# paradigmxyz/reth

Hardware: NVIDIA H100
Metric: keccak256_digests_per_sec (higher is better)
Workload: dtype u64

## Files before the change

reth_b200/csrc/tk_branch.cuh:

```cuda

struct ChildInfo {
    uint32_t id;
    uint32_t nib;
    uint32_t meta;
};

template <bool COHERENT = false>
__device__ __forceinline__ ChildInfo fetch_child(const ForestDev &f, uint32_t j0, uint32_t c) {
    ChildInfo ci;
    if (c == 0) {
        uint32_t g = f.gap_sorted[j0];
        ci.id = f.E[g - 1];
        ci.nib = f.nibs[g] >> 4;
    } else {
        uint32_t g = f.gap_sorted[j0 + c - 1];
        ci.id = f.S[g];
        ci.nib = f.nibs[g] & 15;
    }
    if (COHERENT) ci.meta = ci.id < f.n ? __ldcg(f.leaf_meta + ci.id) : __ldcg(f.node_meta + (ci.id - (uint32_t)f.n));
    else ci.meta = ci.id < f.n ? f.leaf_meta[ci.id] : f.node_meta[ci.id - (uint32_t)f.n];
    return ci;
}

template <class W>
// ... 118 lines not shown
        const uint32_t t3 = (sw & 1) ? (i >= 1 ? T2[i - 1] : 0u) : T2[i];
        if (base_word + i < 34) m[base_word + i] ^= t3;
    }
}

__device__ __forceinline__ void branch23_words(const uint32_t (&r0)[8], const uint32_t (&r1)[8], const uint32_t (&r2)[8], uint32_t n0,
                                               uint32_t n1, uint32_t n2, bool three, uint32_t (&m)[34]) {
#pragma unroll
    for (int w = 0; w < 34; w++) {
        uint32_t two_v = w == 0 ? 0x808051f8u : (w < 20 ? 0x80808080u : (w == 20 ? 0x01808080u : 0u));
        uint32_t three_v = w == 0 ? 0x808071f8u : (w < 28 ? 0x80808080u : (w == 28 ? 0x01808080u : 0u));
        if (w == 33) {
            two_v = 0x80000000u;
            three_v = 0x80000000u;
        }
        m[w] = two_v == three_v ? two_v : (three ? three_v : two_v);
    }
    xor_child33(m, 0, r0, n0, true);
    xor_child33(m, 8, r1, n1, true);
    xor_child33(m, 16, r2, n2, three);
}

template <int BLOCK>
__device__ __forceinline__ uint32_t thread_finish_node(Strip<BLOCK> &s, uint32_t (&ref)[8], uint32_t meta, int pd, int d,
                                                       const uint8_t *key, uint32_t &hashed, uint32_t &exts) {
    if (pd + 1 >= d) return meta;
    s.reset();
    uint32_t elen = encode_extension(s, key, (uint32_t)(pd + 1), (uint32_t)d, ref, meta);
    exts++;
    return strip_to_ref(s, elen, pd < 0, ref, hashed) | META_EXT;
}

template <int BLOCK, int MAXC, bool COHERENT>
__device__ __forceinline__ void thread_build_node(Strip<BLOCK> &s, uint32_t *smem, const ForestDev &f, uint32_t v, int d,
                                                  uint32_t &hashed, uint32_t &exts, uint32_t (&ref)[8]) {
    s.init(smem);
    uint32_t j0 = f.node_start[v], k = f.node_start[v + 1] - j0;
    if (k + 1 > (uint32_t)MAXC) k = MAXC - 1;
    uint32_t state_mask, tree_mask, hash_mask, l, r;
    uint32_t meta;
    bool done = false;
    if constexpr (MAXC == 3 && !COHERENT) {
        const uint32_t n = (uint32_t)f.n;
        const uint32_t g0 = f.gap_sorted[j0], g1 = k >= 2 ? f.gap_sorted[j0 + 1] : g0;
        uint32_t id[3], nb[3], mt[3];
        id[0] = f.E[g0 - 1];
        nb[0] = f.nibs[g0] >> 4;
        id[1] = f.S[g0];
        nb[1] = f.nibs[g0] & 15;
        id[2] = k >= 2 ? f.S[g1] : id[1];
        nb[2] = k >= 2 ? (uint32_t)(f.nibs[g1] & 15) : 15u;
#pragma unroll
        for (int c = 0; c < 3; c++) mt[c] = id[c] < n ? f.leaf_meta[id[c]] : f.node_meta[id[c] - n];
        const bool three = k >= 2;
        if (k >= 1 && ((mt[0] | mt[1] | (three ? mt[2] : 0u)) & META_LEN) == 0) {
            uint32_t rr[3][8];
#pragma unroll
            for (int c = 0; c < 3; c++)
                load32_nc(id[c] < n ? f.leaf_ref + 32 * (uint64_t)id[c] : f.node_ref + 32 * (uint64_t)(id[c] - n), rr[c]);
            state_mask = tree_mask = hash_mask = 0;
#pragma unroll
            for (int c = 0; c < 3; c++) {
                if (c < 2 || three) {
                    const uint32_t bit = 1u << nb[c];
                    state_mask |= bit;
                    if (id[c] >= n || (mt[c] & META_ISNODE)) {
                        if (!(mt[c] & META_EXT)) hash_mask |= bit;
                        if (mt[c] & META_STORED) tree_mask |= bit;
                    }
                }
// ... 4 lines not shown
            uint32_t m[34];
            branch23_words(rr[0], rr[1], rr[2], nb[0], nb[1], nb[2], three, m);
            uint64_t a[25];
#pragma unroll
            for (int q = 0; q < 17; q++) a[q] = ((uint64_t)m[2 * q + 1] << 32) | m[2 * q];
#pragma unroll
            for (int q = 17; q < 25; q++) a[q] = 0;
            keccak_f1600_final(a);
#pragma unroll
            for (int q = 0; q < 4; q++) {
                ref[2 * q] = (uint32_t)a[q];
                ref[2 * q + 1] = (uint32_t)(a[q] >> 32);
            }
            hashed++;
            meta = 0;
            done = true;
        }
    }
    uint32_t len = 0;
    if (!done) len = encode_branch_u<BLOCK, MAXC, COHERENT>(s, f, j0, k, state_mask, tree_mask, hash_mask, l, r);
    const int pd = parent_depth(f, l, r);
    if (!done) meta = strip_to_ref(s, len, pd < 0 && pd + 1 >= d, ref, hashed);
    meta = thread_finish_node(s, ref, meta, pd, d, f.keys + 32 * (uint64_t)l, hashed, exts);
    bool stored = (tree_mask | hash_mask) != 0;
    if (stored) meta |= META_STORED;
    store32(f.node_ref + 32 * (uint64_t)v, ref);
    f.node_meta[v] = (uint8_t)meta;
    f.node_l[v] = l;
    f.node_r[v] = r;
    f.node_masks[v] = make_ushort4((unsigned short)state_mask, (unsigned short)tree_mask, (unsigned short)hash_mask,
                                   (unsigned short)d);
    f.S[l] = (uint32_t)f.n + v;
    f.E[r] = (uint32_t)f.n + v;
}

struct PrefetchedNode3 {
    uint32_t v, j0, k;
    uint32_t g0, g1;
    uint32_t id[3], nb[3], mt[3];
    uint32_t rr[3][8];
    uint32_t nl, nr;
    bool valid;
};

template <int BLOCK>
__device__ __forceinline__ void pf3_stage_a(const ForestDev &f, const uint32_t *__restrict__ node_order, uint64_t p, uint32_t pos_hi,
                                            PrefetchedNode3 &x) {
    x.valid = p < pos_hi;
    if (x.valid) {
        x.v = __ldg(node_order + p);
        x.j0 = f.node_start[x.v];
        x.k = f.node_start[x.v + 1] - x.j0;
    }
}
__device__ __forceinline__ void pf3_stage_b(const ForestDev &f, PrefetchedNode3 &x) {
    if (x.valid) {
        x.g0 = f.gap_sorted[x.j0];
        x.g1 = x.k >= 2 ? f.gap_sorted[x.j0 + 1] : x.g0;
    }
}
__device__ __forceinline__ void pf3_stage_c(const ForestDev &f, PrefetchedNode3 &x) {
    if (x.valid) {
        const uint32_t nib0 = f.nibs[x.g0], nib1 = f.nibs[x.g1];
        x.id[0] = f.E[x.g0 - 1];
        x.id[1] = f.S[x.g0];
        x.id[2] = x.k >= 2 ? f.S[x.g1] : x.id[1];
// ... 70 lines not shown
            keccak_rounds<17, 23>(a);
            keccak_round(a, 0x8000000080008008ULL);
#pragma unroll
            for (int q = 0; q < 4; q++) {
                ref[2 * q] = (uint32_t)a[q];
                ref[2 * q + 1] = (uint32_t)(a[q] >> 32);
            }
            hashed++;
            int pdl = depth_of(lpl), pdr = depth_of(lpr);
            int pd = pdl > pdr ? pdl : pdr;
            meta = thread_finish_node(s, ref, 0u, pd, d, f.keys + 32 * (uint64_t)l, hashed, exts);
            if ((tree_mask | hash_mask) != 0) meta |= META_STORED;
            store32(f.node_ref + 32 * (uint64_t)v, ref);
            f.node_meta[v] = (uint8_t)meta;
            f.node_l[v] = l;
            f.node_r[v] = r;
            f.node_masks[v] = make_ushort4((unsigned short)state_mask, (unsigned short)tree_mask, (unsigned short)hash_mask,
                                           (unsigned short)d);
            f.S[l] = n + v;
            f.E[r] = n + v;
        } else {
            pf3_stage_b(f, nx);
            pf3_stage_c(f, nx);
            pf3_stage_d(f, nx);
            thread_build_node<BLOCK, 3, false>(s, smem, f, v, d, hashed, exts, ref);
        }
        cur = nx;
        p += step;
    }
    flush_counters(f.counters, hashed, exts);
}

template <int BLOCK, int MAXC>
__global__ void __launch_bounds__(BLOCK) branch_kernel(ForestDev f, const uint32_t *__restrict__ node_order,
                                                       uint32_t pos_lo, uint32_t pos_hi, int d) {
    extern __shared__ uint32_t smem[];
    if (*(volatile int *)f.err != B200_DEVERR_NONE) return;
    Strip<BLOCK> s;
    uint32_t hashed = 0, exts = 0;
    const uint32_t step = gridDim.x * BLOCK;
    for (uint64_t p64 = (uint64_t)pos_lo + blockIdx.x * BLOCK + threadIdx.x; p64 < pos_hi; p64 += step) {
        uint32_t ref[8];
        thread_build_node<BLOCK, MAXC, false>(s, smem, f, __ldg(node_order + p64), d, hashed, exts, ref);
    }
    flush_counters(f.counters, hashed, exts);
}
```

reth_b200/csrc/tk_dtrie.cuh:

```cuda

static __device__ __forceinline__ uint32_t dt_nib(const uint8_t *key, uint32_t i) { return key_nibble_mem(key, i); }

static __device__ __forceinline__ uint32_t dt_lcp(const uint8_t *a, const uint8_t *b, uint32_t from, uint32_t limit) {
    uint32_t i = from & ~1u;
    for (; i < limit; i += 2) {
        uint32_t x = a[i >> 1] ^ b[i >> 1];
        if (x) {
            uint32_t l = (x & 0xF0) ? i : i + 1;
            return l < limit ? l : limit;
        }
    }
    return limit;
}

static __device__ __forceinline__ void dt_copy32(uint8_t *dst, const uint8_t *src) {
    const uint4 *s = reinterpret_cast<const uint4 *>(src);
    uint4 *d = reinterpret_cast<uint4 *>(dst);
    d[0] = s[0];
    d[1] = s[1];
}
static __device__ __forceinline__ void dt_copy72(uint8_t *dst, const uint8_t *src) {
    const uint64_t *s = reinterpret_cast<const uint64_t *>(src);
    uint64_t *d = reinterpret_cast<uint64_t *>(dst);
#pragma unroll
// ... 761 lines not shown
                                                     uint32_t &hashed, uint32_t &exts, uint32_t (&ref)[8]) {
    s.init(smem);
    const int d = t.ndepth[v];
    uint32_t state_mask, tree_mask, hash_mask;
    const uint32_t payload = dt_branch_payload<true>(t, v, state_mask, tree_mask, hash_mask);
    dt_put_branch<true>(s, t, v, payload);
    const uint32_t par = t.nparent[v];
    const int pd = par == DT_NONE ? -1 : (int)t.ndepth[par];
    uint32_t meta = strip_to_ref(s, list_header_len(payload) + payload, pd < 0 && pd + 1 >= d, ref, hashed);
    meta = thread_finish_node(s, ref, meta, pd, d, t.nkey + 32 * (uint64_t)v, hashed, exts);
    if ((tree_mask | hash_mask) != 0) meta |= META_STORED;
    if ((t.nmeta[v] & META_STORED) && !(meta & META_STORED)) dt_record_removed(t, v);
    store32(t.nref + 32 * (uint64_t)v, ref);
    t.nmeta[v] = (uint8_t)meta;
    t.nmasks[v] = make_ushort4((unsigned short)state_mask, (unsigned short)tree_mask, (unsigned short)hash_mask, (unsigned short)d);
    t.built[atomicAdd(&t.g[DG_BUILT], 1u)] = v;
}

template <int BLOCK>
__global__ void __launch_bounds__(BLOCK) dt_wavefront_thread_kernel(DTrieDev t, const uint32_t *__restrict__ count_p,
                                                                   uint32_t *__restrict__ handoff_list,
                                                                   uint32_t *__restrict__ handoff_count, int split_depth) {
    extern __shared__ uint32_t smem[];
    if (*(volatile int *)t.err != B200_DEVERR_NONE) return;
    Strip<BLOCK> s;
    uint32_t hashed = 0, exts = 0;
    const uint32_t e = blockIdx.x * BLOCK + threadIdx.x;
    const uint32_t sd = e < *count_p ? t.seeds[e] : DT_NONE;
    if (sd != DT_NONE) {
        uint32_t ref[8];
        uint32_t p;
        if (sd & DT_LEAF) {
            const uint32_t x = sd & ~DT_LEAF;
            s.init(smem);
            p = t.lparent[x];
            const int pd = p == DT_NONE ? -1 : (int)t.ndepth[p];
            uint32_t k[8];
            load32_nc(t.lkey + 32 * (uint64_t)x, k);
            uint32_t len = t.account ? encode_leaf<Strip<BLOCK>, true>(s, k, pd, t.lval + 72 * (uint64_t)x,
                                                                        t.lsroot ? t.lsroot + 32 * (uint64_t)x : nullptr, t.err)
                                     : encode_leaf<Strip<BLOCK>, false>(s, k, pd, t.lval + 32 * (uint64_t)x, nullptr, t.err);
            uint32_t meta = strip_to_ref(s, len, pd < 0, ref, hashed);
            store32(t.lref + 32 * (uint64_t)x, ref);
            t.lmeta[x] = (uint8_t)meta;
        } else {
            dt_thread_build_node<BLOCK>(s, smem, t, sd, hashed, exts, ref);
            p = t.nparent[sd];
        }
        bool top = true;
        for (int hops = 0; p != DT_NONE; hops++) {
            if (hops > DT_MAX_HOPS) {
                atomicExch(t.err, B200_DEVERR_CORRUPT);
                top = false;
                break;
            }
            if ((int)t.ndepth[p] < split_depth) {
                __threadfence();
                handoff_list[atomicAdd(handoff_count, 1u)] = p;
                top = false;
                break;
            }
            __threadfence();
            bool last = atomicSub(&t.npending[p], 1u) == 1u;
            __threadfence();
            if (!last) {
                top = false;
                break;
            }
            dt_thread_build_node<BLOCK>(s, smem, t, p, hashed, exts, ref);
            p = t.nparent[p];
        }
        if (top) store32(t.top_out + (uint64_t)t.top_stride * dt_trie_of(t, sd), ref);
    }
    flush_counters(t.counters, hashed, exts);
}
// ... 56 lines not shown
```

reth_b200/csrc/tk_items.cuh:

```cuda
template <int BLOCK>
__global__ void __launch_bounds__(BLOCK) item_leaf_kernel(ForestDev f, ItemLeavesDev it, const uint8_t *__restrict__ values,
                                                          const uint8_t *__restrict__ storage_roots) {
    extern __shared__ uint32_t smem[];
    if (*(volatile int *)f.err == B200_DEVERR_UNSORTED || *(volatile int *)f.err == B200_DEVERR_BAD_OFFSETS) return;
    Strip<BLOCK> s;
    uint32_t hashed = 0, exts = 0;
    const uint32_t stride = it.account ? (uint32_t)sizeof(b200_account_dev) : 32u;
    const uint64_t step = (uint64_t)gridDim.x * BLOCK;
    for (uint64_t i = (uint64_t)blockIdx.x * BLOCK + threadIdx.x; i < f.n; i += step) {
        s.init(smem);
        const int pd = parent_depth(f, i, i);
        const uint32_t L = it.key_nibs[i];
        uint32_t ref[8], meta;
        if (L >= 64) {
            uint32_t k[8];
            load32(f.keys + 32 * i, k);
            const uint8_t *vp = values + (uint64_t)stride * i;
            uint32_t len = it.account ? encode_leaf<Strip<BLOCK>, true>(s, k, pd, vp, storage_roots ? storage_roots + 32 * i : nullptr, f.err)
                                      : encode_leaf<Strip<BLOCK>, false>(s, k, pd, vp, nullptr, f.err);
            meta = strip_to_ref(s, len, pd < 0, ref, hashed);
        } else {
            if (pd >= (int)L) atomicExch(f.err, B200_DEVERR_UNSORTED);
            {
                const uint2 *q = reinterpret_cast<const uint2 *>(values + (uint64_t)stride * i);
#pragma unroll
                for (int w = 0; w < 4; w++) {
                    uint2 t = __ldg(q + w);
                    ref[2 * w] = t.x;
                    ref[2 * w + 1] = t.y;
                }
            }
            meta = META_ISNODE | ((it.flags[i] & 1) ? META_STORED : 0u) |
                   thread_finish_node(s, ref, 0u, pd, (int)L, f.keys + 32 * i, hashed, exts);
        }
        store32(f.leaf_ref + 32 * i, ref);
        f.leaf_meta[i] = (uint8_t)meta;
        f.S[i] = (uint32_t)i;
        f.E[i] = (uint32_t)i;
    }
    flush_counters(f.counters, hashed, exts);
}

cudaError_t launch_item_leaves(const ForestDev &f, const ItemLeavesDev &it, const uint8_t *values, const uint8_t *storage_roots,
                               cudaStream_t st) {
    if (f.n == 0) return cudaSuccess;
    auto k = item_leaf_kernel<LEAF_BLOCK>;
    size_t smem = (size_t)LEAF_WORDS_ACCOUNT * LEAF_BLOCK * 4;
    k<<<persistent_grid(k, LEAF_BLOCK, smem, f.n), LEAF_BLOCK, smem, st>>>(f, it, values, storage_roots);
    return cudaGetLastError();
}
```

reth_b200/csrc/tk_launchers.cuh:

```cuda

static inline unsigned blocks_for(uint64_t n, unsigned block) { return (unsigned)((n + block - 1) / block); }

static int g_sms = 0;
static int sms() {
    if (!g_sms) {
        int dev = 0;
        cudaGetDevice(&dev);
        cudaDeviceGetAttribute(&g_sms, cudaDevAttrMultiProcessorCount, dev);
        if (g_sms <= 0) g_sms = 132;
    }
    return g_sms;
}

template <typename K>
static unsigned persistent_grid(K kernel, int block, size_t smem, uint64_t work_items) {
    static std::mutex mu;
    static std::unordered_map<const void *, int> cache;
    int per_sm;
    {
        std::lock_guard<std::mutex> g(mu);
        auto it = cache.find((const void *)kernel);
        if (it == cache.end()) {
            cudaFuncSetAttribute(kernel, cudaFuncAttributeMaxDynamicSharedMemorySize, (int)smem);
            per_sm = 1;
// ... 28 lines not shown
    return cudaGetLastError();
}
cudaError_t launch_gap_keys(const uint8_t *Lp, uint64_t G, uint16_t *key, uint32_t *val, uint32_t *unresolved, cudaStream_t st) {
    if (G == 0) return cudaSuccess;
    gap_keys_kernel<<<blocks_for(G, 256), 256, 0, st>>>(Lp, G, key, val, unresolved);
    return cudaGetLastError();
}
cudaError_t launch_bucket_offsets(const uint16_t *key_sorted, uint64_t G, uint32_t *bucket_off, cudaStream_t st) {
    bucket_offsets_kernel<<<1, 96, 0, st>>>(key_sorted, G, bucket_off);
    return cudaGetLastError();
}
cudaError_t launch_head_fix(const uint8_t *keys, uint16_t *key_sorted, const uint32_t *gap_sorted, const uint64_t *seg_offsets,
                            uint64_t n_segs, const uint32_t *unresolved, uint64_t G, cudaStream_t st) {
    if (G == 0) return cudaSuccess;
    head_fix_kernel<<<blocks_for(G, 256), 256, 0, st>>>(keys, key_sorted, gap_sorted, seg_offsets, n_segs, unresolved, G);
    return cudaGetLastError();
}
cudaError_t launch_level_ranges(uint32_t *node_start, const uint32_t *n_nodes_p, const uint32_t *bucket_off,
                                uint32_t *level_lo, cudaStream_t st) {
    level_ranges_kernel<<<1, 96, 0, st>>>(node_start, n_nodes_p, bucket_off, level_lo, node_start);
    return cudaGetLastError();
}

constexpr int LEAF_BLOCK = 128;
constexpr int LEAF_WORDS_STORAGE = 34;
constexpr int LEAF_WORDS_ACCOUNT = 68;
constexpr int BRANCH_BLOCK = 128;
constexpr int BRANCH_WORDS = 136;

cudaError_t launch_leaves(const ForestDev &f, bool account, const uint8_t *values, const uint8_t *storage_roots,
                          cudaStream_t st) {
    if (f.n == 0) return cudaSuccess;
    if (account) {
        auto k = leaf_kernel<LEAF_BLOCK, true>;
        size_t smem = (size_t)LEAF_WORDS_ACCOUNT * LEAF_BLOCK * 4;
        k<<<persistent_grid(k, LEAF_BLOCK, smem, f.n), LEAF_BLOCK, smem, st>>>(f, values, storage_roots);
    } else {
        auto k = leaf_storage_kernel<LEAF_BLOCK>;
        size_t smem = (size_t)LEAF_WORDS_STORAGE * LEAF_BLOCK * 4;
        k<<<blocks_for(f.n, LEAF_BLOCK), LEAF_BLOCK, smem, st>>>(f, values);
    }
    return cudaGetLastError();
}

template <int MAXC, int WORDS>
static cudaError_t launch_branch_class(const ForestDev &f, const uint32_t *node_order, uint32_t pos_lo, uint32_t pos_hi,
                                       int d, cudaStream_t st) {
    auto k = branch_kernel<BRANCH_BLOCK, MAXC>;
    size_t smem = (size_t)WORDS * BRANCH_BLOCK * 4;
    k<<<persistent_grid(k, BRANCH_BLOCK, smem, pos_hi - pos_lo), BRANCH_BLOCK, smem, st>>>(f, node_order, pos_lo,
                                                                                          pos_hi, d);
    return cudaGetLastError();
}

cudaError_t launch_branch_level(const ForestDev &f, const uint32_t *node_order, uint32_t pos_lo, uint32_t pos_hi,
                                int d, int cls, cudaStream_t st) {
    if (pos_hi <= pos_lo) return cudaSuccess;
    if (cls < 0) {
        constexpr int WARPS = 4;
        uint32_t cnt = pos_hi - pos_lo;
        unsigned blocks = (cnt + WARPS - 1) / WARPS;
        unsigned cap = (unsigned)sms() * 16;
        branch_warp_kernel<WARPS><<<blocks < cap ? blocks : cap, WARPS * 32, 0, st>>>(f, node_order, pos_lo, pos_hi, d);
        return cudaGetLastError();
    }
    switch (cls) {
        case 0: {
            auto k = branch3_pipelined_kernel<BRANCH_BLOCK>;
            size_t smem = (size_t)34 * BRANCH_BLOCK * 4;
// ... 220 lines not shown
```

reth_b200/csrc/tk_leaf.cuh:

```cuda

template <class W, bool ACCOUNT>
__device__ __forceinline__ uint32_t encode_leaf(W &s, const uint32_t (&k)[8], int pd, const uint8_t *val_ptr,
                                                const uint8_t *sroot_ptr, int *err) {
    uint32_t p = (uint32_t)(pd + 1);
    uint32_t m = 64 - p;
    uint32_t hp_len = 1 + (m >> 1);
    uint32_t hp_str = hp_len == 1 ? 1 : 1 + hp_len;
    uint32_t first = (p & 1) ? (0x30u | (byte_at(k, p >> 1) & 15)) : 0x20u;
    uint32_t b0 = (p + 1) >> 1;

    if (!ACCOUNT) {
        uint32_t v[8];
        load32(val_ptr, v);
        uint32_t z = leading_zero_bytes(v);
        if (z == 32) {
            atomicExch(err, B200_DEVERR_ZERO_VALUE);
            z = 31;
        }
        uint32_t vb = 32 - z;
        uint32_t fb = byte_at(v, z);
        bool single = vb == 1 && fb < 0x80;
        uint32_t rlp_v = single ? 1 : 1 + vb;
        uint32_t val_str = single ? 1 : 1 + rlp_v;
        uint32_t payload = hp_str + val_str;
        put_list_header(s, payload);
        if (hp_len > 1) s.byte(0x80 + hp_len);
        s.byte(first);
        s.tail32(k, b0);
        if (single) {
            s.byte(fb);
        } else {
            s.byte(0x80 + rlp_v);
            s.byte(0x80 + vb);
            s.tail32(v, z);
        }
        return list_header_len(payload) + payload;
    } else {
        const uint64_t *ap = reinterpret_cast<const uint64_t *>(val_ptr);
        uint64_t nonce = __ldg(ap);
        uint32_t bal[8], code[8], sroot[8];
        {
            const uint2 *q = reinterpret_cast<const uint2 *>(val_ptr + 8);
#pragma unroll
            for (int i = 0; i < 4; i++) {
                uint2 t = __ldg(q + i);
                bal[2 * i] = t.x;
                bal[2 * i + 1] = t.y;
            }
#pragma unroll
            for (int i = 0; i < 4; i++) {
                uint2 t = __ldg(q + 4 + i);
                code[2 * i] = t.x;
                code[2 * i + 1] = t.y;
            }
        }
        if (sroot_ptr) {
            load32_nc(sroot_ptr, sroot);
        } else {
            sroot[0] = 0x171fe856u; sroot[1] = 0xa655cc1bu; sroot[2] = 0xe64583ffu; sroot[3] = 0x6ef8c092u;
            sroot[4] = 0x1be0485bu; sroot[5] = 0xc0ad6c99u; sroot[6] = 0xb52f6201u; sroot[7] = 0x21b463e3u;
        }
        uint32_t nn = nonce == 0 ? 0 : (8 - (__clzll((long long)nonce) >> 3));
        uint32_t nonce_rlp = (nn == 0 || (nn == 1 && nonce < 0x80)) ? 1 : 1 + nn;
        uint32_t bz = leading_zero_bytes(bal);
        uint32_t bb = 32 - bz;
        uint32_t bfb = bb ? byte_at(bal, bz) : 0;
        uint32_t bal_rlp = (bb == 0 || (bb == 1 && bfb < 0x80)) ? 1 : 1 + bb;
        uint32_t inner_payload = nonce_rlp + bal_rlp + 66;
        uint32_t inner_total = 2 + inner_payload;
        uint32_t payload = hp_str + 2 + inner_total;
        s.byte(0xf8);
        s.byte(payload);
        if (hp_len > 1) s.byte(0x80 + hp_len);
        s.byte(first);
        s.tail32(k, b0);
        s.byte(0xb8);
        s.byte(inner_total);
        s.byte(0xf8);
        s.byte(inner_payload);
        if (nn == 0) {
            s.byte(0x80);
        } else {
            if (nonce_rlp > 1) s.byte(0x80 + nn);
            for (int i = (int)nn - 1; i >= 0; i--) s.byte((uint32_t)(nonce >> (8 * i)) & 0xff);
        }
        if (bb == 0) {
            s.byte(0x80);
        } else if (bal_rlp == 1) {
            s.byte(bfb);
        } else {
            s.byte(0x80 + bb);
            s.tail32(bal, bz);
        }
        s.byte(0xa0);
        s.words8(sroot);
        s.byte(0xa0);
        s.words8(code);
        return 2 + payload;
    }
// ... 53 lines not shown
    X[0] = (two ? 0u : (X[0] & 0xFF000000u)) | A;

    const uint32_t ov = a + 32 - b0, bv8 = 8 * (ov & 3), rel = (ov >> 2) - 5;
    uint32_t T0[13], T1[13];
#pragma unroll
    for (int i = 0; i < 13; i++) T0[i] = i < 10 ? __funnelshift_l(Y[i], Y[i + 1], bv8) : 0u;
#pragma unroll
    for (int i = 0; i < 13; i++) T1[i] = (rel & 2) ? (i >= 2 ? T0[i - 2] : 0u) : T0[i];
#pragma unroll
    for (int i = 0; i < 5; i++) mw[i] = X[i];
#pragma unroll
    for (int i = 0; i < 13; i++) {
        const uint32_t t2 = (rel & 1) ? (i >= 1 ? T1[i - 1] : 0u) : T1[i];
        mw[5 + i] = (5 + i < 9 ? X[5 + i] : 0u) | t2;
    }
    return (two ? 2u : 1u) + payload;
}

__device__ __forceinline__ void keccak_single_block18(const uint32_t (&mw)[18], uint32_t (&dig)[8]) {
    uint64_t a[25];
#pragma unroll
    for (int l = 0; l < 9; l++) a[l] = ((uint64_t)mw[2 * l + 1] << 32) | mw[2 * l];
#pragma unroll
    for (int l = 9; l < 25; l++) a[l] = 0;
    a[16] = 0x8000000000000000ULL;
    keccak_f1600_sparse_final(a);
#pragma unroll
    for (int l = 0; l < 4; l++) {
        dig[2 * l] = (uint32_t)a[l];
        dig[2 * l + 1] = (uint32_t)(a[l] >> 32);
    }
}

template <int BLOCK>
__device__ __forceinline__ uint32_t strip_to_ref(Strip<BLOCK> &s, uint32_t len, bool force_hash, uint32_t (&ref)[8],
                                                 uint32_t &hashed) {
    if (len >= 32 || force_hash) {
        uint32_t blocks = s.finish();
        strip_keccak(s, blocks, ref);
        hashed++;
        return 0;
    }
    while (s.nb != 0) s.byte(0);
#pragma unroll
    for (int i = 0; i < 8; i++) ref[i] = (uint32_t)i < s.nw ? s.read_word(i) : 0;
    return len;
}

template <int BLOCK, bool ACCOUNT>
__global__ void __launch_bounds__(BLOCK) leaf_kernel(ForestDev f, const uint8_t *__restrict__ values,
                                                     const uint8_t *__restrict__ storage_roots) {
    extern __shared__ uint32_t smem[];
    if (*(volatile int *)f.err == B200_DEVERR_UNSORTED || *(volatile int *)f.err == B200_DEVERR_BAD_OFFSETS) return;
    Strip<BLOCK> s;
    uint32_t hashed = 0;
    const uint64_t step = (uint64_t)gridDim.x * BLOCK;
    for (uint64_t i = (uint64_t)blockIdx.x * BLOCK + threadIdx.x; i < f.n; i += step) {
        s.init(smem);
        uint32_t k[8];
        load32(f.keys + 32 * i, k);
        const int pd = parent_depth(f, i, i);
        const uint8_t *vp = ACCOUNT ? values + (uint64_t)sizeof(b200_account_dev) * i : values + 32 * i;
        const uint8_t *sp = (ACCOUNT && storage_roots) ? storage_roots + 32 * i : nullptr;
        uint32_t len = encode_leaf<Strip<BLOCK>, ACCOUNT>(s, k, pd, vp, sp, f.err);
        uint32_t ref[8];
        uint32_t meta = strip_to_ref(s, len, pd < 0, ref, hashed);
        store32(f.leaf_ref + 32 * i, ref);
        f.leaf_meta[i] = (uint8_t)meta;
        f.S[i] = (uint32_t)i;
        f.E[i] = (uint32_t)i;
    }
    for (int o = 16; o; o >>= 1) hashed += __shfl_xor_sync(0xffffffffu, hashed, o);
    if ((threadIdx.x & 31) == 0 && hashed) atomicAdd(&f.counters[CNT_HASHED], (unsigned long long)hashed);
}

template <int BLOCK>
__global__ void __launch_bounds__(BLOCK) leaf_storage_kernel(ForestDev f, const uint8_t *__restrict__ values) {
    extern __shared__ uint32_t smem[];
    __shared__ uint32_t s_hashed;
    if (*(volatile int *)f.err == B200_DEVERR_UNSORTED || *(volatile int *)f.err == B200_DEVERR_BAD_OFFSETS) return;
    if (threadIdx.x == 0) s_hashed = 0;
    __syncthreads();
    const uint64_t i = (uint64_t)blockIdx.x * BLOCK + threadIdx.x;
    uint32_t hashed = 0;
    if (i < f.n) {
        uint32_t k[8], v[8], ref[8];
        load32(f.keys + 32 * i, k);
        load32(values + 32 * i, v);
        const int pd = parent_depth(f, i, i);
        uint32_t meta;
        if (pd >= 0 && pd <= 26) {
            uint32_t zi = 8, zword = 0;
#pragma unroll
            for (int w = 7; w >= 0; w--)
                if (v[w] != 0) {
                    zi = (uint32_t)w;
                    zword = v[w];
                }
            uint32_t z = 4 * zi + ((uint32_t)(__ffs((int)zword) - 1) >> 3);
            if (zi == 8) {
                atomicExch(f.err, B200_DEVERR_ZERO_VALUE);
                z = 31;
            }
            uint32_t mw[18];
            const uint32_t len = storage_leaf_words(k, v, (uint32_t)(pd + 1), z, mw);
            if (len >= 32) {
                keccak_single_block18(mw, ref);
                hashed = 1;
                meta = 0;
            } else {
#pragma unroll
                for (int w = 0; w < 8; w++) ref[w] = (uint32_t)w == (len >> 2) ? (mw[w] & ~(0xFFu << (8 * (len & 3)))) : mw[w];
                meta = len;
            }
        } else {
            Strip<BLOCK> s;
            s.init(smem);
            uint32_t len = encode_leaf<Strip<BLOCK>, false>(s, k, pd, values + 32 * i, nullptr, f.err);
            meta = strip_to_ref(s, len, pd < 0, ref, hashed);
        }
        store32(f.leaf_ref + 32 * i, ref);
        f.leaf_meta[i] = (uint8_t)meta;
        f.S[i] = (uint32_t)i;
        f.E[i] = (uint32_t)i;
    }
    for (int o = 16; o; o >>= 1) hashed += __shfl_xor_sync(0xffffffffu, hashed, o);
    if ((threadIdx.x & 31) == 0 && hashed) atomicAdd(&s_hashed, hashed);
    __syncthreads();
    if (threadIdx.x == 0 && s_hashed) atomicAdd(&f.counters[CNT_HASHED], (unsigned long long)s_hashed);
}
```

reth_b200/csrc/tk_strip.cuh:

```cuda

template <int BLOCK>
struct Strip {
    uint32_t *w;
    uint32_t prev;
    uint32_t nb;
    uint32_t nw;
    __device__ __forceinline__ void init(uint32_t *smem) {
        w = smem + threadIdx.x;
        prev = 0;
        nb = 0;
        nw = 0;
    }
    __device__ __forceinline__ void byte(uint32_t b) {
        prev = (prev >> 8) | (b << 24);
        if (++nb == 4) {
            w[nw * BLOCK] = prev;
            nw++;
            nb = 0;
        }
    }
    __device__ __forceinline__ void word(uint32_t x) {
        w[nw * BLOCK] = __funnelshift_rc(prev, x, 32 - 8 * nb);
        nw++;
        prev = x;
// ... 94 lines not shown
static __device__ __forceinline__ int parent_depth(const ForestDev &f, uint64_t l, uint64_t r) {
    const int pdl = depth_of(f.Lp[l]), pdr = depth_of(f.Lp[r + 1]);
    return pdl > pdr ? pdl : pdr;
}

static __device__ __forceinline__ void flush_warp_counters(unsigned long long *counters, uint32_t hashed, uint32_t exts) {
    if ((threadIdx.x & 31) == 0) {
        if (hashed) atomicAdd(&counters[CNT_HASHED], (unsigned long long)hashed);
        if (exts) atomicAdd(&counters[CNT_EXT], (unsigned long long)exts);
    }
}
static __device__ __forceinline__ void flush_counters(unsigned long long *counters, uint32_t hashed, uint32_t exts) {
    for (int o = 16; o; o >>= 1) {
        hashed += __shfl_xor_sync(0xffffffffu, hashed, o);
        exts += __shfl_xor_sync(0xffffffffu, exts, o);
    }
    flush_warp_counters(counters, hashed, exts);
}

static __device__ __forceinline__ uint32_t leading_zero_bytes(const uint32_t (&x)[8]) {
    uint32_t z = 32;
#pragma unroll
    for (int i = 7; i >= 0; i--)
        if (x[i] != 0) z = 4u * i + ((__ffs(x[i]) - 1) >> 3);
    return z;
}
static __device__ __forceinline__ uint32_t byte_at(const uint32_t (&x)[8], uint32_t j) {
    uint32_t w = 0;
#pragma unroll
    for (int i = 0; i < 8; i++)
        if ((j >> 2) == (uint32_t)i) w = x[i];
    return (w >> (8 * (j & 3))) & 0xff;
}

struct LinBuf {
    uint8_t *p;
    uint32_t n;
    __device__ __forceinline__ void byte(uint32_t b) { p[n++] = (uint8_t)b; }
    __device__ __forceinline__ void word(uint32_t x) {
        p[n++] = (uint8_t)x;
        p[n++] = (uint8_t)(x >> 8);
        p[n++] = (uint8_t)(x >> 16);
        p[n++] = (uint8_t)(x >> 24);
    }
    __device__ __forceinline__ void words8(const uint32_t (&x)[8]) {
#pragma unroll
        for (int i = 0; i < 8; i++) word(x[i]);
    }
    __device__ __forceinline__ void tail32(const uint32_t (&x)[8], uint32_t b0) {
        for (uint32_t b = b0; b < 32; b++) byte(byte_at(x, b));
    }
};
struct CountBuf {
    uint32_t n;
    __device__ __forceinline__ void byte(uint32_t) { n++; }
    __device__ __forceinline__ void word(uint32_t) { n += 4; }
    __device__ __forceinline__ void words8(const uint32_t (&)[8]) { n += 32; }
    __device__ __forceinline__ void tail32(const uint32_t (&)[8], uint32_t b0) { n += 32 - b0; }
};

template <class W>
static __device__ __forceinline__ void put_list_header(W &s, uint32_t payload) {
    if (payload < 56) {
        s.byte(0xc0 + payload);
    } else if (payload < 256) {
        s.byte(0xf8);
// ... 29 lines not shown
```

reth_b200/csrc/tk_wavefront.cuh:

```cuda

__global__ void mark_pending_kernel(ForestDev f, const uint32_t *__restrict__ idx, uint64_t m,
                                    const uint32_t *__restrict__ leaf_parent, const uint32_t *__restrict__ node_parent,
                                    uint32_t *__restrict__ pending) {
    if (*(volatile int *)f.err != B200_DEVERR_NONE) return;
    uint64_t t = (uint64_t)blockIdx.x * blockDim.x + threadIdx.x;
    if (t >= m) return;
    uint32_t p = leaf_parent[idx[t]];
    while (p != 0xFFFFFFFFu) {
        if (atomicAdd(&pending[p], 1u) != 0u) break;
        p = node_parent[p];
    }
}

__device__ __forceinline__ bool warp_climb(const ForestDev &f, uint32_t p, const uint32_t *__restrict__ node_parent,
                                           uint32_t *__restrict__ pending, uint32_t *__restrict__ dirty_list,
                                           uint32_t *__restrict__ dirty_count, uint8_t *buf, const WarpKeccak &kw, int lane,
                                           uint32_t &hashed, uint32_t &exts, uint32_t (&out)[8]) {
    while (p != 0xFFFFFFFFu) {
        uint32_t last = 0;
        if (lane == 0) {
            __threadfence();
            last = atomicSub(&pending[p], 1u) == 1u;
            __threadfence();
        }
// ... 35 lines not shown
        if (new_sroots && sroots) {
            uint32_t r[8];
            load32(new_sroots + 32 * t, r);
            store32(sroots + 32 * (uint64_t)i, r);
        }
    }
    uint32_t out[8];
    warp_leaf_ref(true, buf, f.keys + 32 * (uint64_t)i, parent_depth(f, i, i), new_accts + 72 * t,
                  sroots ? (new_sroots ? new_sroots + 32 * t : sroots + 32 * (uint64_t)i) : nullptr, f.err, kw, lane, hashed, out);
    if (lane == 0) {
        store32(f.leaf_ref + 32 * (uint64_t)i, out);
        f.leaf_meta[i] = 0;
    }
    __syncwarp();
    bool top = warp_climb(f, leaf_parent[i], node_parent, pending, dirty_list, dirty_count, buf, kw, lane, hashed, exts, out);
    if (top && lane == 0) store32(root_out, out);
    flush_warp_counters(f.counters, hashed, exts);
}

template <int BLOCK>
__global__ void __launch_bounds__(BLOCK) wavefront_thread_kernel(
    ForestDev f, uint8_t *__restrict__ accts, uint8_t *__restrict__ sroots, const uint8_t *__restrict__ new_accts,
    const uint8_t *__restrict__ new_sroots, const uint32_t *__restrict__ idx, uint64_t m,
    const uint32_t *__restrict__ leaf_parent, const uint32_t *__restrict__ node_parent, uint32_t *__restrict__ pending,
    uint32_t *__restrict__ dirty_list, uint32_t *__restrict__ dirty_count, uint32_t *__restrict__ handoff_list,
    uint32_t *__restrict__ handoff_count, uint8_t *__restrict__ root_out, int split_depth) {
    extern __shared__ uint32_t smem[];
    if (*(volatile int *)f.err != B200_DEVERR_NONE) return;
    Strip<BLOCK> s;
    uint32_t hashed = 0, exts = 0;
    uint64_t t = (uint64_t)blockIdx.x * BLOCK + threadIdx.x;
    if (t < m) {
        const uint32_t i = idx[t];
        s.init(smem);
        {
            const uint64_t *src = reinterpret_cast<const uint64_t *>(new_accts + 72 * t);
            uint64_t *dst = reinterpret_cast<uint64_t *>(accts + 72 * (uint64_t)i);
#pragma unroll
            for (int w = 0; w < 9; w++) dst[w] = src[w];
            if (new_sroots && sroots) {
                uint32_t r[8];
                load32(new_sroots + 32 * t, r);
                store32(sroots + 32 * (uint64_t)i, r);
            }
        }
        uint32_t k[8];
        load32(f.keys + 32 * (uint64_t)i, k);
        const int pd = parent_depth(f, i, i);
        uint32_t len = encode_leaf<Strip<BLOCK>, true>(
            s, k, pd, new_accts + 72 * t, sroots ? (new_sroots ? new_sroots + 32 * t : sroots + 32 * (uint64_t)i) : nullptr,
            f.err);
        uint32_t ref[8];
        uint32_t meta = strip_to_ref(s, len, pd < 0, ref, hashed);
        store32(f.leaf_ref + 32 * (uint64_t)i, ref);
        f.leaf_meta[i] = (uint8_t)meta;
        uint32_t p = leaf_parent[i];
        bool top = true;
        while (p != 0xFFFFFFFFu) {
            int d = f.node_masks[p].w;
            if (d < split_depth) {
                __threadfence();
                handoff_list[atomicAdd(handoff_count, 1u)] = p;
                top = false;
                break;
            }
            __threadfence();
            bool last = atomicSub(&pending[p], 1u) == 1u;
            __threadfence();
            if (!last) {
                top = false;
                break;
            }
            thread_build_node<BLOCK, 16, true>(s, smem, f, p, d, hashed, exts, ref);
            dirty_list[atomicAdd(dirty_count, 1u)] = p;
            p = node_parent[p];
        }
        if (top) store32(root_out, ref);
    }
    flush_counters(f.counters, hashed, exts);
}

template <int WARPS>
__global__ void __launch_bounds__(WARPS * 32) climb_kernel(ForestDev f, const uint32_t *__restrict__ start_list,
                                                          const uint32_t *__restrict__ start_count_p,
                                                          const uint32_t *__restrict__ node_parent,
                                                          uint32_t *__restrict__ pending, uint32_t *__restrict__ dirty_list,
// ... 17 lines not shown
```

Measured before the change: 3.978 billion.

## Software-pipeline node_order and node_start loads in branch_kernel, add min-blocks launch bounds

```diff
diff --git a/reth_b200/csrc/tk_branch.cuh b/reth_b200/csrc/tk_branch.cuh
--- a/reth_b200/csrc/tk_branch.cuh
+++ b/reth_b200/csrc/tk_branch.cuh
@@ -174,10 +174,9 @@
 }
 
 template <int BLOCK, int MAXC, bool COHERENT>
-__device__ __forceinline__ void thread_build_node(Strip<BLOCK> &s, uint32_t *smem, const ForestDev &f, uint32_t v, int d,
-                                                  uint32_t &hashed, uint32_t &exts, uint32_t (&ref)[8]) {
+__device__ __forceinline__ void thread_build_node_at(Strip<BLOCK> &s, uint32_t *smem, const ForestDev &f, uint32_t v, uint32_t j0,
+                                                     uint32_t k, int d, uint32_t &hashed, uint32_t &exts, uint32_t (&ref)[8]) {
     s.init(smem);
-    uint32_t j0 = f.node_start[v], k = f.node_start[v + 1] - j0;
     if (k + 1 > (uint32_t)MAXC) k = MAXC - 1;
     uint32_t state_mask, tree_mask, hash_mask, l, r;
     uint32_t meta;
@@ -248,6 +247,12 @@
                                    (unsigned short)d);
     f.S[l] = (uint32_t)f.n + v;
     f.E[r] = (uint32_t)f.n + v;
+}
+template <int BLOCK, int MAXC, bool COHERENT>
+__device__ __forceinline__ void thread_build_node(Strip<BLOCK> &s, uint32_t *smem, const ForestDev &f, uint32_t v, int d,
+                                                  uint32_t &hashed, uint32_t &exts, uint32_t (&ref)[8]) {
+    const uint32_t j0 = f.node_start[v];
+    thread_build_node_at<BLOCK, MAXC, COHERENT>(s, smem, f, v, j0, f.node_start[v + 1] - j0, d, hashed, exts, ref);
 }
 
 struct PrefetchedNode3 {
@@ -384,16 +389,35 @@
 }
 
 template <int BLOCK, int MAXC>
-__global__ void __launch_bounds__(BLOCK) branch_kernel(ForestDev f, const uint32_t *__restrict__ node_order,
-                                                       uint32_t pos_lo, uint32_t pos_hi, int d) {
+__global__ void __launch_bounds__(BLOCK, MAXC > 12 ? 3 : (MAXC > 7 ? 4 : 5))
+    branch_kernel(ForestDev f, const uint32_t *__restrict__ node_order, uint32_t pos_lo, uint32_t pos_hi, int d) {
     extern __shared__ uint32_t smem[];
     if (*(volatile int *)f.err != B200_DEVERR_NONE) return;
     Strip<BLOCK> s;
     uint32_t hashed = 0, exts = 0;
     const uint32_t step = gridDim.x * BLOCK;
-    for (uint64_t p64 = (uint64_t)pos_lo + blockIdx.x * BLOCK + threadIdx.x; p64 < pos_hi; p64 += step) {
+    uint64_t p64 = (uint64_t)pos_lo + blockIdx.x * BLOCK + threadIdx.x;
+    uint32_t v = p64 < pos_hi ? __ldg(node_order + p64) : 0u;
+    uint32_t j0 = 0, k = 0;
+    if (p64 < pos_hi) {
+        j0 = f.node_start[v];
+        k = f.node_start[v + 1] - j0;
+    }
+    uint32_t v1 = p64 + step < pos_hi ? __ldg(node_order + p64 + step) : 0u;
+    for (; p64 < pos_hi; p64 += step) {
+        const bool more1 = p64 + step < pos_hi, more2 = p64 + 2 * (uint64_t)step < pos_hi;
+        const uint32_t v2 = more2 ? __ldg(node_order + p64 + 2 * (uint64_t)step) : 0u;
+        uint32_t j0n = 0, kn = 0;
+        if (more1) {
+            j0n = f.node_start[v1];
+            kn = f.node_start[v1 + 1] - j0n;
+        }
         uint32_t ref[8];
-        thread_build_node<BLOCK, MAXC, false>(s, smem, f, __ldg(node_order + p64), d, hashed, exts, ref);
+        thread_build_node_at<BLOCK, MAXC, false>(s, smem, f, v, j0, k, d, hashed, exts, ref);
+        v = v1;
+        j0 = j0n;
+        k = kn;
+        v1 = v2;
     }
     flush_counters(f.counters, hashed, exts);
 }
```

Result: no change. 3.963 billion, median of 6 (-0.4%).

## Build account leaf RLP in registers and hash directly, bypassing shared strip

Applied to the files above, without the earlier changes.

```diff
diff --git a/reth_b200/csrc/tk_dtrie.cuh b/reth_b200/csrc/tk_dtrie.cuh
--- a/reth_b200/csrc/tk_dtrie.cuh
+++ b/reth_b200/csrc/tk_dtrie.cuh
@@ -817,15 +817,12 @@
         uint32_t p;
         if (sd & DT_LEAF) {
             const uint32_t x = sd & ~DT_LEAF;
-            s.init(smem);
             p = t.lparent[x];
             const int pd = p == DT_NONE ? -1 : (int)t.ndepth[p];
             uint32_t k[8];
             load32_nc(t.lkey + 32 * (uint64_t)x, k);
-            uint32_t len = t.account ? encode_leaf<Strip<BLOCK>, true>(s, k, pd, t.lval + 72 * (uint64_t)x,
-                                                                        t.lsroot ? t.lsroot + 32 * (uint64_t)x : nullptr, t.err)
-                                     : encode_leaf<Strip<BLOCK>, false>(s, k, pd, t.lval + 32 * (uint64_t)x, nullptr, t.err);
-            uint32_t meta = strip_to_ref(s, len, pd < 0, ref, hashed);
+            uint32_t meta = leaf_to_ref<BLOCK>(s, smem, t.account, k, pd, t.lval + (t.account ? 72 : 32) * (uint64_t)x,
+                                               t.lsroot ? t.lsroot + 32 * (uint64_t)x : nullptr, t.err, ref, hashed);
             store32(t.lref + 32 * (uint64_t)x, ref);
             t.lmeta[x] = (uint8_t)meta;
         } else {
diff --git a/reth_b200/csrc/tk_items.cuh b/reth_b200/csrc/tk_items.cuh
--- a/reth_b200/csrc/tk_items.cuh
+++ b/reth_b200/csrc/tk_items.cuh
@@ -16,9 +16,8 @@
             uint32_t k[8];
             load32(f.keys + 32 * i, k);
             const uint8_t *vp = values + (uint64_t)stride * i;
-            uint32_t len = it.account ? encode_leaf<Strip<BLOCK>, true>(s, k, pd, vp, storage_roots ? storage_roots + 32 * i : nullptr, f.err)
-                                      : encode_leaf<Strip<BLOCK>, false>(s, k, pd, vp, nullptr, f.err);
-            meta = strip_to_ref(s, len, pd < 0, ref, hashed);
+            meta = leaf_to_ref<BLOCK>(s, smem, it.account, k, pd, vp, storage_roots ? storage_roots + 32 * i : nullptr, f.err,
+                                      ref, hashed);
         } else {
             if (pd >= (int)L) atomicExch(f.err, B200_DEVERR_UNSORTED);
             {
diff --git a/reth_b200/csrc/tk_launchers.cuh b/reth_b200/csrc/tk_launchers.cuh
--- a/reth_b200/csrc/tk_launchers.cuh
+++ b/reth_b200/csrc/tk_launchers.cuh
@@ -84,9 +84,9 @@
                           cudaStream_t st) {
     if (f.n == 0) return cudaSuccess;
     if (account) {
-        auto k = leaf_kernel<LEAF_BLOCK, true>;
+        auto k = leaf_account_kernel<LEAF_BLOCK>;
         size_t smem = (size_t)LEAF_WORDS_ACCOUNT * LEAF_BLOCK * 4;
-        k<<<persistent_grid(k, LEAF_BLOCK, smem, f.n), LEAF_BLOCK, smem, st>>>(f, values, storage_roots);
+        k<<<blocks_for(f.n, LEAF_BLOCK), LEAF_BLOCK, smem, st>>>(f, values, storage_roots);
     } else {
         auto k = leaf_storage_kernel<LEAF_BLOCK>;
         size_t smem = (size_t)LEAF_WORDS_STORAGE * LEAF_BLOCK * 4;
diff --git a/reth_b200/csrc/tk_leaf.cuh b/reth_b200/csrc/tk_leaf.cuh
--- a/reth_b200/csrc/tk_leaf.cuh
+++ b/reth_b200/csrc/tk_leaf.cuh
@@ -1,3 +1,27 @@
+
+__device__ __forceinline__ void load_account(const uint8_t *val_ptr, const uint8_t *sroot_ptr, uint64_t &nonce,
+                                             uint32_t (&bal)[8], uint32_t (&code)[8], uint32_t (&sroot)[8]) {
+    nonce = __ldg(reinterpret_cast<const uint64_t *>(val_ptr));
+    const uint2 *q = reinterpret_cast<const uint2 *>(val_ptr + 8);
+#pragma unroll
+    for (int i = 0; i < 4; i++) {
+        uint2 t = __ldg(q + i);
+        bal[2 * i] = t.x;
+        bal[2 * i + 1] = t.y;
+    }
+#pragma unroll
+    for (int i = 0; i < 4; i++) {
+        uint2 t = __ldg(q + 4 + i);
+        code[2 * i] = t.x;
+        code[2 * i + 1] = t.y;
+    }
+    if (sroot_ptr) {
+        load32_nc(sroot_ptr, sroot);
+    } else {
+        sroot[0] = 0x171fe856u; sroot[1] = 0xa655cc1bu; sroot[2] = 0xe64583ffu; sroot[3] = 0x6ef8c092u;
+        sroot[4] = 0x1be0485bu; sroot[5] = 0xc0ad6c99u; sroot[6] = 0xb52f6201u; sroot[7] = 0x21b463e3u;
+    }
+}
 
 template <class W, bool ACCOUNT>
 __device__ __forceinline__ uint32_t encode_leaf(W &s, const uint32_t (&k)[8], int pd, const uint8_t *val_ptr,
@@ -6,7 +30,7 @@
     uint32_t m = 64 - p;
     uint32_t hp_len = 1 + (m >> 1);
     uint32_t hp_str = hp_len == 1 ? 1 : 1 + hp_len;
-    uint32_t first = (p & 1) ? (0x30u | (byte_at(k, p >> 1) & 15)) : 0x20u;
+    uint32_t first = (p & 1) ? (0x30u | ((ACCOUNT ? byte_at_sel(k, p >> 1) : byte_at(k, p >> 1)) & 15)) : 0x20u;
     uint32_t b0 = (p + 1) >> 1;
 
     if (!ACCOUNT) {
@@ -36,35 +60,14 @@
         }
         return list_header_len(payload) + payload;
     } else {
-        const uint64_t *ap = reinterpret_cast<const uint64_t *>(val_ptr);
-        uint64_t nonce = __ldg(ap);
+        uint64_t nonce;
         uint32_t bal[8], code[8], sroot[8];
-        {
-            const uint2 *q = reinterpret_cast<const uint2 *>(val_ptr + 8);
-#pragma unroll
-            for (int i = 0; i < 4; i++) {
-                uint2 t = __ldg(q + i);
-                bal[2 * i] = t.x;
-                bal[2 * i + 1] = t.y;
-            }
-#pragma unroll
-            for (int i = 0; i < 4; i++) {
-                uint2 t = __ldg(q + 4 + i);
-                code[2 * i] = t.x;
-                code[2 * i + 1] = t.y;
-            }
-        }
-        if (sroot_ptr) {
-            load32_nc(sroot_ptr, sroot);
-        } else {
-            sroot[0] = 0x171fe856u; sroot[1] = 0xa655cc1bu; sroot[2] = 0xe64583ffu; sroot[3] = 0x6ef8c092u;
-            sroot[4] = 0x1be0485bu; sroot[5] = 0xc0ad6c99u; sroot[6] = 0xb52f6201u; sroot[7] = 0x21b463e3u;
-        }
+        load_account(val_ptr, sroot_ptr, nonce, bal, code, sroot);
         uint32_t nn = nonce == 0 ? 0 : (8 - (__clzll((long long)nonce) >> 3));
         uint32_t nonce_rlp = (nn == 0 || (nn == 1 && nonce < 0x80)) ? 1 : 1 + nn;
         uint32_t bz = leading_zero_bytes(bal);
         uint32_t bb = 32 - bz;
-        uint32_t bfb = bb ? byte_at(bal, bz) : 0;
+        uint32_t bfb = bb ? byte_at_sel(bal, bz) : 0;
         uint32_t bal_rlp = (bb == 0 || (bb == 1 && bfb < 0x80)) ? 1 : 1 + bb;
         uint32_t inner_payload = nonce_rlp + bal_rlp + 66;
         uint32_t inner_total = 2 + inner_payload;
@@ -184,6 +187,98 @@
     }
 }
 
+template <int LEVELS, int NIN, int NOUT>
+__device__ __forceinline__ void bytes_down(const uint32_t (&in)[NIN], uint32_t s, uint32_t (&out)[NOUT]) {
+    uint32_t w[NIN];
+#pragma unroll
+    for (int j = 0; j < NIN; j++) w[j] = in[j];
+    const uint32_t sw = s >> 2, sb8 = 8 * (s & 3);
+#pragma unroll
+    for (int l = LEVELS - 1; l >= 0; l--) {
+#pragma unroll
+        for (int j = 0; j < NIN; j++) w[j] = (sw & (1u << l)) ? (j + (1 << l) < NIN ? w[j + (1 << l)] : 0u) : w[j];
+    }
+#pragma unroll
+    for (int j = 0; j < NOUT; j++) out[j] = __funnelshift_r(j < NIN ? w[j] : 0u, j + 1 < NIN ? w[j + 1] : 0u, sb8);
+}
+
+__device__ __forceinline__ uint32_t account_leaf_words(const uint32_t (&k)[8], uint64_t nonce, const uint32_t (&bal)[8],
+                                                       const uint32_t (&sroot)[8], const uint32_t (&code)[8], uint32_t p,
+                                                       uint32_t (&mw)[38]) {
+    const uint32_t b0 = (p + 1) >> 1;
+    const uint32_t hp_len = 33 - b0;
+    const uint32_t kb = p >> 1;
+    const uint32_t kw = kb < 4 ? k[0] : (kb < 8 ? k[1] : (kb < 12 ? k[2] : k[3]));
+    const uint32_t first = (p & 1) ? (0x30u | ((kw >> (8 * (kb & 3))) & 15u)) : 0x20u;
+
+    const uint32_t nn = nonce == 0 ? 0 : (8 - (__clzll((long long)nonce) >> 3));
+    const bool n_single = nn == 0 || (nn == 1 && nonce < 0x80);
+    const uint32_t nf = n_single ? 1 : 1 + nn;
+    const uint64_t nbe = ((uint64_t)__byte_perm((uint32_t)nonce, 0, 0x0123) << 32) | __byte_perm((uint32_t)(nonce >> 32), 0, 0x0123);
+    const uint64_t nsig = nbe >> (8 * (8 - (nn ? nn : 1)));
+    const uint64_t nfld = nn == 0 ? 0x80u : (n_single ? nonce : ((0x80u + nn) | (nsig << 8)));
+
+    const uint32_t bz = leading_zero_bytes(bal);
+    const bool b_single = bz == 31 && (bal[7] >> 24) < 0x80;
+    const uint32_t hb = b_single ? 0 : 1;
+    const uint32_t bf = b_single ? 1 : 33 - bz;
+
+    const uint32_t inner_payload = nf + bf + 66;
+    const uint32_t payload = hp_len + 5 + inner_payload;
+    const uint32_t ob = 40 - b0 + nf;
+
+    uint32_t KU[13], X[13];
+    KU[0] = 0;
+#pragma unroll
+    for (int j = 0; j < 8; j++) KU[j + 1] = k[j];
+    KU[9] = 0xb8u | ((inner_payload + 2) << 8) | (0xf8u << 16) | (inner_payload << 24);
+    KU[10] = (uint32_t)nfld;
+    KU[11] = (uint32_t)(nfld >> 32);
+    KU[12] = nn == 8 ? (uint32_t)(nsig >> 56) : 0u;
+    bytes_down<2>(KU, b0, X);
+    X[0] = 0xf8u | (payload << 8) | ((0x80u + hp_len) << 16) | (first << 24);
+    const uint32_t hdr = b_single ? 0u : 0x80u + 32 - bz;
+#pragma unroll
+    for (int j = 6; j < 13; j++) X[j] |= (uint32_t)j == (ob >> 2) ? hdr << (8 * (ob & 3)) : 0u;
+
+    uint32_t RU[38], Y[38];
+#pragma unroll
+    for (int j = 0; j < 13; j++) RU[j] = 0;
+#pragma unroll
+    for (int j = 0; j < 8; j++) RU[13 + j] = bal[j];
+    RU[21] = 0xa0u | (sroot[0] << 8);
+#pragma unroll
+    for (int j = 1; j < 8; j++) RU[21 + j] = __funnelshift_l(sroot[j - 1], sroot[j], 8);
+    RU[29] = (sroot[7] >> 24) | (0xa0u << 8) | (code[0] << 16);
+#pragma unroll
+    for (int j = 1; j < 8; j++) RU[29 + j] = __funnelshift_l(code[j - 1], code[j], 16);
+    RU[37] = (code[7] >> 16) | (1u << 16);
+    bytes_down<4>(RU, 52 + bz - hb - ob, Y);
+#pragma unroll
+    for (int j = 0; j < 38; j++) mw[j] = (j < 13 ? X[j] : 0u) | Y[j];
+    return 2 + payload;
+}
+
+__device__ __forceinline__ void keccak_leaf_words38(const uint32_t (&mw)[38], uint32_t len, uint32_t (&dig)[8]) {
+    uint64_t a[25];
+#pragma unroll
+    for (int l = 0; l < 17; l++) a[l] = ((uint64_t)mw[2 * l + 1] << 32) | mw[2 * l];
+#pragma unroll
+    for (int l = 17; l < 25; l++) a[l] = 0;
+    if (len >= 136) {
+        keccak_f1600(a);
+#pragma unroll
+        for (int l = 0; l < 2; l++) a[l] ^= ((uint64_t)mw[35 + 2 * l] << 32) | mw[34 + 2 * l];
+    }
+    a[16] ^= 0x8000000000000000ULL;
+    keccak_f1600_final(a);
+#pragma unroll
+    for (int l = 0; l < 4; l++) {
+        dig[2 * l] = (uint32_t)a[l];
+        dig[2 * l + 1] = (uint32_t)(a[l] >> 32);
+    }
+}
+
 template <int BLOCK>
 __device__ __forceinline__ uint32_t strip_to_ref(Strip<BLOCK> &s, uint32_t len, bool force_hash, uint32_t (&ref)[8],
                                                  uint32_t &hashed) {
@@ -199,31 +294,82 @@
     return len;
 }
 
-template <int BLOCK, bool ACCOUNT>
-__global__ void __launch_bounds__(BLOCK) leaf_kernel(ForestDev f, const uint8_t *__restrict__ values,
-                                                     const uint8_t *__restrict__ storage_roots) {
+__device__ __forceinline__ uint32_t storage_leaf_ref(const uint32_t (&k)[8], const uint32_t (&v)[8], int pd, int *err,
+                                                     uint32_t (&ref)[8], uint32_t &hashed) {
+    uint32_t zi = 8, zword = 0;
+#pragma unroll
+    for (int w = 7; w >= 0; w--)
+        if (v[w] != 0) {
+            zi = (uint32_t)w;
+            zword = v[w];
+        }
+    uint32_t z = 4 * zi + ((uint32_t)(__ffs((int)zword) - 1) >> 3);
+    if (zi == 8) {
+        atomicExch(err, B200_DEVERR_ZERO_VALUE);
+        z = 31;
+    }
+    uint32_t mw[18];
+    const uint32_t len = storage_leaf_words(k, v, (uint32_t)(pd + 1), z, mw);
+    if (len >= 32) {
+        keccak_single_block18(mw, ref);
+        hashed++;
+        return 0;
+    }
+#pragma unroll
+    for (int w = 0; w < 8; w++) ref[w] = (uint32_t)w == (len >> 2) ? (mw[w] & ~(0xFFu << (8 * (len & 3)))) : mw[w];
+    return len;
+}
+
+template <int BLOCK>
+__device__ __forceinline__ uint32_t leaf_to_ref(Strip<BLOCK> &s, uint32_t *smem, bool account, const uint32_t (&k)[8],
+                                                int pd, const uint8_t *val_ptr, const uint8_t *sroot_ptr, int *err,
+                                                uint32_t (&ref)[8], uint32_t &hashed) {
+    if (account && pd >= 0 && pd <= 29) {
+        uint64_t nonce;
+        uint32_t bal[8], code[8], sroot[8], mw[38];
+        load_account(val_ptr, sroot_ptr, nonce, bal, code, sroot);
+        const uint32_t len = account_leaf_words(k, nonce, bal, sroot, code, (uint32_t)(pd + 1), mw);
+        keccak_leaf_words38(mw, len, ref);
+        hashed++;
+        return 0;
+    }
+    if (!account && pd >= 0 && pd <= 26) {
+        uint32_t v[8];
+        load32(val_ptr, v);
+        return storage_leaf_ref(k, v, pd, err, ref, hashed);
+    }
+    s.init(smem);
+    const uint32_t len = account ? encode_leaf<Strip<BLOCK>, true>(s, k, pd, val_ptr, sroot_ptr, err)
+                                 : encode_leaf<Strip<BLOCK>, false>(s, k, pd, val_ptr, nullptr, err);
+    return strip_to_ref(s, len, pd < 0, ref, hashed);
+}
+
+template <int BLOCK>
+__global__ void __launch_bounds__(BLOCK) leaf_account_kernel(ForestDev f, const uint8_t *__restrict__ values,
+                                                             const uint8_t *__restrict__ storage_roots) {
     extern __shared__ uint32_t smem[];
+    __shared__ uint32_t s_hashed;
     if (*(volatile int *)f.err == B200_DEVERR_UNSORTED || *(volatile int *)f.err == B200_DEVERR_BAD_OFFSETS) return;
-    Strip<BLOCK> s;
+    if (threadIdx.x == 0) s_hashed = 0;
+    __syncthreads();
+    const uint64_t i = (uint64_t)blockIdx.x * BLOCK + threadIdx.x;
     uint32_t hashed = 0;
-    const uint64_t step = (uint64_t)gridDim.x * BLOCK;
-    for (uint64_t i = (uint64_t)blockIdx.x * BLOCK + threadIdx.x; i < f.n; i += step) {
-        s.init(smem);
-        uint32_t k[8];
+    if (i < f.n) {
+        uint32_t k[8], ref[8];
         load32(f.keys + 32 * i, k);
         const int pd = parent_depth(f, i, i);
-        const uint8_t *vp = ACCOUNT ? values + (uint64_t)sizeof(b200_account_dev) * i : values + 32 * i;
-        const uint8_t *sp = (ACCOUNT && storage_roots) ? storage_roots + 32 * i : nullptr;
-        uint32_t len = encode_leaf<Strip<BLOCK>, ACCOUNT>(s, k, pd, vp, sp, f.err);
-        uint32_t ref[8];
-        uint32_t meta = strip_to_ref(s, len, pd < 0, ref, hashed);
+        Strip<BLOCK> s;
+        const uint32_t meta = leaf_to_ref<BLOCK>(s, smem, true, k, pd, values + (uint64_t)sizeof(b200_account_dev) * i,
+                                                 storage_roots ? storage_roots + 32 * i : nullptr, f.err, ref, hashed);
         store32(f.leaf_ref + 32 * i, ref);
         f.leaf_meta[i] = (uint8_t)meta;
         f.S[i] = (uint32_t)i;
         f.E[i] = (uint32_t)i;
     }
     for (int o = 16; o; o >>= 1) hashed += __shfl_xor_sync(0xffffffffu, hashed, o);
-    if ((threadIdx.x & 31) == 0 && hashed) atomicAdd(&f.counters[CNT_HASHED], (unsigned long long)hashed);
+    if ((threadIdx.x & 31) == 0 && hashed) atomicAdd(&s_hashed, hashed);
+    __syncthreads();
+    if (threadIdx.x == 0 && s_hashed) atomicAdd(&f.counters[CNT_HASHED], (unsigned long long)s_hashed);
 }
 
 template <int BLOCK>
@@ -242,29 +388,7 @@
         const int pd = parent_depth(f, i, i);
         uint32_t meta;
         if (pd >= 0 && pd <= 26) {
-            uint32_t zi = 8, zword = 0;
-#pragma unroll
-            for (int w = 7; w >= 0; w--)
-                if (v[w] != 0) {
-                    zi = (uint32_t)w;
-                    zword = v[w];
-                }
-            uint32_t z = 4 * zi + ((uint32_t)(__ffs((int)zword) - 1) >> 3);
-            if (zi == 8) {
-                atomicExch(f.err, B200_DEVERR_ZERO_VALUE);
-                z = 31;
-            }
-            uint32_t mw[18];
-            const uint32_t len = storage_leaf_words(k, v, (uint32_t)(pd + 1), z, mw);
-            if (len >= 32) {
-                keccak_single_block18(mw, ref);
-                hashed = 1;
-                meta = 0;
-            } else {
-#pragma unroll
-                for (int w = 0; w < 8; w++) ref[w] = (uint32_t)w == (len >> 2) ? (mw[w] & ~(0xFFu << (8 * (len & 3)))) : mw[w];
-                meta = len;
-            }
+            meta = storage_leaf_ref(k, v, pd, f.err, ref, hashed);
         } else {
             Strip<BLOCK> s;
             s.init(smem);
diff --git a/reth_b200/csrc/tk_strip.cuh b/reth_b200/csrc/tk_strip.cuh
--- a/reth_b200/csrc/tk_strip.cuh
+++ b/reth_b200/csrc/tk_strip.cuh
@@ -150,6 +150,13 @@
         if ((j >> 2) == (uint32_t)i) w = x[i];
     return (w >> (8 * (j & 3))) & 0xff;
 }
+static __device__ __forceinline__ uint32_t byte_at_sel(const uint32_t (&x)[8], uint32_t j) {
+    const uint32_t q = j >> 2;
+    const uint32_t a0 = (q & 1) ? x[1] : x[0], a1 = (q & 1) ? x[3] : x[2];
+    const uint32_t a2 = (q & 1) ? x[5] : x[4], a3 = (q & 1) ? x[7] : x[6];
+    const uint32_t w = (q & 4) ? ((q & 2) ? a3 : a2) : ((q & 2) ? a1 : a0);
+    return (w >> (8 * (j & 3))) & 0xff;
+}
 
 struct LinBuf {
     uint8_t *p;
diff --git a/reth_b200/csrc/tk_wavefront.cuh b/reth_b200/csrc/tk_wavefront.cuh
--- a/reth_b200/csrc/tk_wavefront.cuh
+++ b/reth_b200/csrc/tk_wavefront.cuh
@@ -91,7 +91,6 @@
     uint64_t t = (uint64_t)blockIdx.x * BLOCK + threadIdx.x;
     if (t < m) {
         const uint32_t i = idx[t];
-        s.init(smem);
         {
             const uint64_t *src = reinterpret_cast<const uint64_t *>(new_accts + 72 * t);
             uint64_t *dst = reinterpret_cast<uint64_t *>(accts + 72 * (uint64_t)i);
@@ -106,11 +105,10 @@
         uint32_t k[8];
         load32(f.keys + 32 * (uint64_t)i, k);
         const int pd = parent_depth(f, i, i);
-        uint32_t len = encode_leaf<Strip<BLOCK>, true>(
-            s, k, pd, new_accts + 72 * t, sroots ? (new_sroots ? new_sroots + 32 * t : sroots + 32 * (uint64_t)i) : nullptr,
-            f.err);
         uint32_t ref[8];
-        uint32_t meta = strip_to_ref(s, len, pd < 0, ref, hashed);
+        uint32_t meta = leaf_to_ref<BLOCK>(
+            s, smem, true, k, pd, new_accts + 72 * t,
+            sroots ? (new_sroots ? new_sroots + 32 * t : sroots + 32 * (uint64_t)i) : nullptr, f.err, ref, hashed);
         store32(f.leaf_ref + 32 * (uint64_t)i, ref);
         f.leaf_meta[i] = (uint8_t)meta;
         uint32_t p = leaf_parent[i];
```

Result: no change. 3.953 billion before, 3.953 billion after, median of 6 (+0.0%).
